# xbpeng/DeepMimic

Measured on NVIDIA H100. Metric: env-steps/sec (30 Hz policy steps; humanoid3d_spinkick, 4096 envs/GPU), higher is better.
Workload: dtype f32

## Files before the change

### deepmimic_b200/csrc/kernels/dm_step.cu

```cuda
#include "dm_model.cuh"
#include <type_traits>

namespace dmk {

namespace {

template <int W>
struct Tl {
    static __device__ __forceinline__ float shfl(float v, int src) { return __shfl_sync(0xffffffffu, v, src, W); }
    static __device__ __forceinline__ int shfli(int v, int src) { return __shfl_sync(0xffffffffu, v, src, W); }
    static __device__ __forceinline__ V3 shfl3(V3 v, int src) { return mk3(shfl(v.x, src), shfl(v.y, src), shfl(v.z, src)); }
    static __device__ __forceinline__ S6 shfl6(S6 v, int src) { return mks(shfl3(v.a, src), shfl3(v.l, src)); }
};
__device__ __forceinline__ void ld12(const float* p, float* o) {
    const float4 a = reinterpret_cast<const float4*>(p)[0], b = reinterpret_cast<const float4*>(p)[1], c_ = reinterpret_cast<const float4*>(p)[2];
    o[0] = a.x; o[1] = a.y; o[2] = a.z; o[3] = a.w; o[4] = b.x; o[5] = b.y; o[6] = b.z; o[7] = b.w; o[8] = c_.x; o[9] = c_.y; o[10] = c_.z; o[11] = c_.w;
}
__device__ __forceinline__ void st12(float* p, const float* o) {
    reinterpret_cast<float4*>(p)[0] = make_float4(o[0], o[1], o[2], o[3]); reinterpret_cast<float4*>(p)[1] = make_float4(o[4], o[5], o[6], o[7]);
    reinterpret_cast<float4*>(p)[2] = make_float4(o[8], o[9], o[10], o[11]);
}
__device__ __forceinline__ float rcp_fast(float x) { float r; asm("rcp.approx.ftz.f32 %0, %1;" : "=f"(r) : "f"(x)); return r; }
__device__ __forceinline__ int wmax(int v) {
#pragma unroll
// ... 31 lines not shown
__device__ __forceinline__ V3 quat_rotvec3(Q4 q) {
    float s = sqrtf(q.x * q.x + q.y * q.y + q.z * q.z);
    if (!(s > 0.000001f)) return mk3(0.f, 0.f, 0.f);
    float th = normalize_angle3(2.0f * atan2f(s, q.w));
    float k = th / s;
    return mk3(q.x * k, q.y * k, q.z * k);
}
__device__ __forceinline__ Q4 quat_integrate3(V3 omega, Q4 quat, bool base_body, float dt) {
    V3 angvel = base_body ? omega : qrot(quat, omega);
    float fAngle = sqrtf(dot(angvel, angvel));
    const float kThr = 0.5f * 1.57079632679489661923f;
    if (fAngle * dt > kThr) fAngle = kThr / dt;
    V3 axis;
    if (fAngle < 0.001f) axis = angvel * __fmaf_rn(-fAngle, (dt * dt * dt) * 0.020833333333f * fAngle, 0.5f * dt);
    else axis = angvel * (__sinf(0.5f * fAngle * dt) / fAngle);
    float cw = __cosf(fAngle * dt * 0.5f);
    Q4 r = base_body ? qmul(quat, mkq(-axis.x, -axis.y, -axis.z, cw)) : qmul(mkq(axis.x, axis.y, axis.z, cw), quat);
    float n = rsqrtf(r.x * r.x + r.y * r.y + r.z * r.z + r.w * r.w);
    return mkq(r.x * n, r.y * n, r.z * n, r.w * n);
}

enum LkSlot { kLC = 0 , kLM = 3,
              kLD = 4 , kLThr = 7,
              kLWd = 8 , kLInt = 14 , kLInt2 = 15 ,
              kLWb = 16 , kLFlg = 22 , kLTree = 23 ,
              kLAx = 24 , kLTl = 27,
              kLZr = 28 ,
              kLHe = 32 , kLKp = 35,
              kLKd = 36, kLLo = 37, kLHi = 38, kLChild = 39 ,
              kLDc = 40 , kLMc = 43 ,
              kLDyn = 44 , kLDChild = 45 ,
              kLkFloats = 48 };
__device__ __forceinline__ float4 ld4(const float* p) { return *reinterpret_cast<const float4*>(p); }
enum HdrSlot { kHLayout = 0, kHLvc = 24, kHGrav = 32 , kHh = 35, kHScale = 36, kHMu = 37, kHFdt = 38, kHDmax = 39 , kHdrFloats = 40 };
__device__ __forceinline__ float* step_smem() { extern __shared__ __align__(16) float dm_step_sm[]; return dm_step_sm; }

}

int dm_step_layout(int nl, int n, int chain_len, int maxrows, int W, StepLayout* L) {
    const int maxpts = maxrows / 3;
    int o = 0;
    L->nl = nl; L->n = n; L->chain_len = chain_len; L->maxrows = maxrows; L->maxpts = maxpts;
    L->oU = o; o += nl * 24;
    L->oR = o; o += nl * 12;
    L->oA = o;
    const int world = nl * 24, tri = maxrows * (maxrows + 1) / 2;
    L->oW = o; L->oV = o + nl * 12;
    L->oPp = o + world; L->oQ = L->oPp + maxpts * 4;
    const int pre = world + maxpts * 4 + 4 * 8;
    o += (pre > tri ? pre : tri);
    o = (o + 3) & ~3;
    const int ys = dm_step_y_stride(W), scr = 28 * (nl - 1);
    L->oY = o; o += (chain_len * ys > scr) ? chain_len * ys : scr;
    L->oLam = o; o += maxrows; o += (o & 1); L->oRhs = o; o += maxrows; L->oInv = o; o += maxrows;
    L->oRl = o; o += maxrows;
    L->oPi = o; o += maxpts; L->oPr = o; o += maxpts;
    L->oG = o; o += 21 + 13 + 2;
    L->oZ = o; o += ((n + 3) / 4) * 4;
    L->env_floats = ((o + 15) / 32) * 32 + 16;
    L->hot_floats = kHdrFloats + ((nl * kLkFloats + (nl * nl + nl * chain_len + 3) / 4 + 3) / 4) * 4;
    return L->hot_floats * 4 + 0;
}
int dm_step_smem_bytes(const StepLayout& L, int tiles) { return (L.hot_floats + L.env_floats * tiles) * static_cast<int>(sizeof(float)); }

constexpr int kSubstepBarriers = 2;
constexpr int kPgsBlock = 2;
enum PgsSection { kSecLimit = 0, kSecNormal = 1, kSecFriction = 2 };
// ... 64 lines not shown
            for (int k = 0; k < B; ++k) ao[s][k] = a_own(s, ik[k], tk[k]);
#pragma unroll
        for (int k = 0; k < B; ++k) {
            float sel = w[0];
#pragma unroll
            for (int s = 1; s < S; ++s) if (ik[k] >= s * W) sel = w[s];
            wk[k] = T::shfl(sel, (S == 1) ? ik[k] : (ik[k] & (W - 1)));
        }
#pragma unroll
        for (int k = 0; k < B; ++k) {
            float c = fmaxf(fmaf(-inv[k], wk[k], rhs[k]), lo[k] - lam[k]);
            if (SEC != kSecNormal) c = fminf(c, hi[k] - lam[k]);
            c = vk[k] ? c : 0.f;
#pragma unroll
            for (int j = k + 1; j < B; ++j) wk[j] = fmaf(ain[j * (j - 1) / 2 + k], c, wk[j]);
            if (vk[k] && writer[k]) sLam[ik[k]] = (SEC == kSecNormal) ? fmaxf(lam[k] + c, 0.f) : fminf(fmaxf(lam[k] + c, lo[k]), hi[k]);
#pragma unroll
            for (int s = 0; s < S; ++s) w[s] = fmaf(ao[s][k], c, w[s]);
        }
        __syncwarp();
    };
#pragma unroll 1
    for (int it = 0; it < 10; ++it) {
#pragma unroll 1
        for (int p0 = 0; p0 < NLmax; p0 += B) block(p0, it, std::integral_constant<int, kSecLimit>{});
#pragma unroll 1
        for (int p0 = 0; p0 < Pmax; p0 += B) block(p0, it, std::integral_constant<int, kSecNormal>{});
#pragma unroll 1
        for (int p0 = 0; p0 < 2 * Pmax; p0 += B) block(p0, it, std::integral_constant<int, kSecFriction>{});
    }
}

template <int W>
__device__ __noinline__ void solve_rows(int NL, int P, float* mani, int alive, unsigned int* prf) {
    using T = Tl<W>;
    float* const sm_ = step_smem();
    const int* LYS = reinterpret_cast<const int*>(sm_ + kHLayout);
    const float* LK = sm_ + kHdrFloats;
    const int lane = threadIdx.x % W;
    const float h = sm_[kHh], mu = sm_[kHMu];
#ifdef DM_PROFILE
    unsigned int pt = static_cast<unsigned int>(clock64());
#define SPROF(sec) do { if ((threadIdx.x & 31) == 0) { unsigned int t_ = static_cast<unsigned int>(clock64()); prf[sec] += t_ - pt; pt = t_; } } while (0)
#else
#define SPROF(sec) do { } while (0)
#endif
    const StepLayout& LY = *reinterpret_cast<const StepLayout*>(LYS);
    const int nl = LY.nl, CL = LY.chain_len, MR = LY.maxrows;
    constexpr int YS = dm_step_y_stride(W);
    float* const E = sm_ + LY.hot_floats + (threadIdx.x / W) * LY.env_floats;
    const unsigned char* CD = reinterpret_cast<const unsigned char*>(LK + nl * kLkFloats);
    const unsigned char* CH = CD + nl * nl;
    float* sU = E + LY.oU; float* sS = E + LY.oR; float* sW = E + LY.oW; float* sV = E + LY.oV; float* sA = E + LY.oA; float* sY = E + LY.oY;
    float* sLam = E + LY.oLam; float2* sRI = reinterpret_cast<float2*>(E + LY.oRhs); int* sRl = reinterpret_cast<int*>(E + LY.oRl);
    float* sPp = E + LY.oPp; float* sPi = E + LY.oPi; int* sPr = reinterpret_cast<int*>(E + LY.oPr);
    float* sQ = E + LY.oQ; float* sG = E + LY.oG; float* sZ = E + LY.oZ;
    auto lk_i = [&](int j) { return reinterpret_cast<const int*>(LK + j * kLkFloats)[kLInt]; };
    auto lk_i2 = [&](int j) { return reinterpret_cast<const int*>(LK + j * kLkFloats)[kLInt2]; };
    auto shift_f = [](S6 f, V3 c) { return mks(f.a + cross(c, f.l), f.l); };
    const int NR = NL + 3 * P;
    const int NRmax = (W == 32) ? NR : wmax(NR);
    const int nslots = (NRmax + W - 1) / W;
    constexpr int kSlots = 2;
#pragma unroll
    for (int s = 0; s < kSlots; ++s) {
        const int rid = lane + s * W;
        if (s < nslots) {
            const bool rv_ = rid < NR;
            int b = 0, kind = 0 , p = 0;
            float lsign = 1.f, lpen = 0.f;
            if (rv_) {
                if (rid < NL) { b = __float_as_int(sQ[rid]); lsign = sQ[8 + rid]; lpen = sQ[16 + rid]; }
                else if (rid < NL + P) { kind = 1; p = rid - NL; b = sPr[p] >> 2; }
                else { const int f = rid - NL - P; p = f >> 1; kind = 2 + (f & 1); b = sPr[p] >> 2; }
                sRl[rid] = b;
            }
            S6 f = mks(mk3(0, 0, 0), mk3(0, 0, 0));
            float rvel = 0.f, pdist = 0.f;
            if (rv_ && kind != 0) {
                const float* w = sW + b * 12;
                pdist = sPp[p * 4 + 3];
                const V3 rel = mk3(sPp[p * 4] - w[9], sPp[p * 4 + 1] - w[10], sPp[p * 4 + 2] - w[11]);
                const V3 fl_ = (kind == 1) ? mk3(0.f, 1.f, 0.f) : ((kind == 2) ? mk3(-1.f, 0.f, 0.f) : mk3(0.f, 0.f, 1.f));
                f = mks(cross(rel, fl_), fl_);
                const float* v = sV + b * 12;
                rvel = dot(fl_, mk3(v[3], v[4], v[5]) + cross(mk3(v[0], v[1], v[2]), rel));
            }
            float acc = 0.f;
            int cur = b;
            bool first = true;
#pragma unroll 1
            while (true) {
                const int info = lk_i(cur);
                const int par = static_cast<int>(static_cast<signed char>(info & 0xff)), nd = (info >> 16) & 0xff, dp0 = (info >> 24) & 0xff;
                const float4* u4 = reinterpret_cast<const float4*>(sU + cur * 24);
                const float4* q4 = reinterpret_cast<const float4*>(sS + cur * 12);
                const float4 ua = u4[0], ub = u4[1], uc = u4[2], ud = u4[3], ue = u4[4], uf = u4[5];
                const float4 qa = q4[0], qb = q4[1], qc = q4[2];
                if (nd == 3) {
// ... 31 lines not shown
            {
                float x[6] = {f.a.x, f.a.y, f.a.z, f.l.x, f.l.y, f.l.z};
                int o = 0;
#pragma unroll
                for (int i = 0; i < 6; ++i) {
#pragma unroll
                    for (int k = 0; k < i; ++k) x[i] -= sG[o++] * x[k];
                    x[i] *= sG[15 + i];
                    if (rv_) sY[i * YS + rid] = x[i];
                    acc += x[i] * x[i];
                }
            }
            if (rv_) {
                const float inv = acc > 1.1920929e-7f ? 1.0f / acc : 0.f;
                float rhs, lam0 = 0.f;
                if (kind == 1) {
                    float perr = 0.f, verr = -rvel;
                    if (pdist > 0.f) verr -= pdist / h; else perr = -pdist * 0.2f / h;
                    rhs = perr * inv + verr * inv;
                    lam0 = sPi[p] * 0.85f;
                } else if (kind != 0) rhs = -rvel * inv;
                else {
                    float perr = 0.f, verr = -rvel;
                    const bool combine = lpen > -0.04f;
                    if (lpen > 0.f) verr = -lpen / h; else perr = -lpen * 0.2f / h;
                    rhs = combine ? (perr * inv + verr * inv) : (verr * inv);
                }
                sRI[rid] = make_float2(rhs, inv); sLam[rid] = lam0;
            }
        }
    }
    __syncwarp();
    SPROF(7);
    const int Pmax = (W == 32) ? P : wmax(P);
    const int NLmax = (W == 32) ? NL : wmax(NL);
    {
        constexpr int kSq2 = (W == 16) ? 22 : 36;
        const int region = max(nl * 24, MR * (MR + 1) / 2);
        const int mode = (nslots == 1) ? 0 : ((NRmax <= kSq2 && kSq2 * kSq2 + W <= region) ? 1 : 2);
        const int st = (mode == 0) ? W : kSq2;
        auto put = [&](int i, int j, float v) {
            if (mode != 2) { sA[i * st + j] = v; sA[j * st + i] = v; }
            else { const int hi_ = max(i, j), lo_ = min(i, j); sA[hi_ * (hi_ + 1) / 2 + lo_] = v; }
        };
#pragma unroll 1
        for (int j = 0; j < NLmax; ++j) {
            const bool jv = j < NL;
            const int bj = jv ? sRl[j] : 0;
#pragma unroll 1
            for (int i0 = 0; i0 < NRmax; i0 += W) {
                const int i = i0 + lane;
                const bool pv = jv && i < NR && i >= j;
                const int cd = pv ? CD[sRl[i] * nl + bj] : 0;
                const float* yi = sY + (pv ? i : 0); const float* yj = sY + (jv ? j : 0);
                float acc = 0.f;
#pragma unroll 1
                for (int k = 0; k < CL; k += 4, yi += 4 * YS, yj += 4 * YS) {
                    const float a0 = yi[0], a1 = yi[YS], a2 = yi[2 * YS], a3 = yi[3 * YS];
                    const float b0 = yj[0], b1 = yj[YS], b2 = yj[2 * YS], b3 = yj[3 * YS];
                    if (k < cd) acc += a0 * b0;
                    if (k + 1 < cd) acc += a1 * b1;
                    if (k + 2 < cd) acc += a2 * b2;
                    if (k + 3 < cd) acc += a3 * b3;
                }
                if (pv) put(i, j, acc);
            }
        }
        const int npp = P * (P + 1) / 2, nppmax = Pmax * (Pmax + 1) / 2;
#pragma unroll 1
        for (int q0 = 0; q0 < nppmax; q0 += W) {
            const int q = q0 + lane;
            const bool pv = q < npp;
            int pp = static_cast<int>((sqrtf(8.0f * static_cast<float>(q) + 1.0f) - 1.0f) * 0.5f);
            if (pp * (pp + 1) / 2 > q) --pp;
            if ((pp + 1) * (pp + 2) / 2 <= q) ++pp;
            const int pr = q - pp * (pp + 1) / 2;
            const int in_p = pv ? NL + pp : 0, it_p = pv ? NL + P + 2 * pp : 0, in_r = pv ? NL + pr : 0, it_r = pv ? NL + P + 2 * pr : 0;
            const int cd = pv ? CD[sRl[in_p] * nl + sRl[in_r]] : 0;
            const float* ypn = sY + in_p; const float* ypt = sY + it_p; const float* yrn = sY + in_r; const float* yrt = sY + it_r;
            float acc[3][3];
#pragma unroll
            for (int x = 0; x < 3; ++x)
#pragma unroll
                for (int y = 0; y < 3; ++y) acc[x][y] = 0.f;
#pragma unroll 1
            for (int k = 0; k < CL; k += 4, ypn += 4 * YS, ypt += 4 * YS, yrn += 4 * YS, yrt += 4 * YS) {
                float av[3][4], bv[3][4];
#pragma unroll
                for (int d = 0; d < 4; ++d) {
                    av[0][d] = ypn[d * YS]; av[1][d] = ypt[d * YS]; av[2][d] = ypt[d * YS + 1];
                    bv[0][d] = yrn[d * YS]; bv[1][d] = yrt[d * YS]; bv[2][d] = yrt[d * YS + 1];
                }
#pragma unroll
                for (int d = 0; d < 4; ++d)
                    if (k + d < cd) {
#pragma unroll
                        for (int x = 0; x < 3; ++x)
#pragma unroll
                            for (int y = 0; y < 3; ++y) acc[x][y] += av[x][d] * bv[y][d];
                    }
            }
            if (pv) {
                if (mode != 2) {
                    float* rp[3] = {sA + in_p * st, sA + it_p * st, sA + it_p * st + st};
                    float* rr[3] = {sA + in_r * st, sA + it_r * st, sA + it_r * st + st};
                    const int cp[3] = {in_p, it_p, it_p + 1}, cr[3] = {in_r, it_r, it_r + 1};
#pragma unroll
                    for (int x = 0; x < 3; ++x)
#pragma unroll
                        for (int y = 0; y < 3; ++y) { rp[x][cr[y]] = acc[x][y]; rr[y][cp[x]] = acc[x][y]; }
                } else {
#pragma unroll
                    for (int x = 0; x < 3; ++x)
#pragma unroll
                        for (int y = 0; y < 3; ++y) put(x == 0 ? in_p : it_p + x - 1, y == 0 ? in_r : it_r + y - 1, acc[x][y]);
                }
            }
        }
        __syncwarp();
        SPROF(8);
        if (mode == 0) pgs_sweeps<W, 1, W, kPgsBlock>(sA, sLam, sRI, lane, NL, P, NLmax, Pmax, mu);
        else if (mode == 1) pgs_sweeps<W, kSlots, kSq2, kPgsBlock>(sA, sLam, sRI, lane, NL, P, NLmax, Pmax, mu);
        else pgs_sweeps<W, kSlots, 0, kPgsBlock>(sA, sLam, sRI, lane, NL, P, NLmax, Pmax, mu);
    }
    SPROF(9);
#pragma unroll 1
    for (int p = lane; p < P; p += W) {
        if (alive) {
            const int ref = sPr[p];
            float* mpt = mani + (ref >> 2) * kManifoldFloats + (ref & 3) * 12;
            mpt[7] = sLam[NL + p]; mpt[8] = sLam[NL + P + 2 * p]; mpt[9] = sLam[NL + P + 2 * p + 1];
        }
    }
    {
        const int info = (lane < nl) ? lk_i(lane) : 0;
        const int nd = (info >> 16) & 0xff, dp0 = (info >> 24) & 0xff;
        const int d0 = (lane < nl) ? (lk_i2(lane) & 0xff) : 0;
        float z0 = 0.f, z1 = 0.f, z2 = 0.f, zb = 0.f;
        const int kb = (lane < 6) ? lane : 0;
        const bool mine = lane < nl && nd > 0;
        const int need = dp0 + nd - 1;
        const unsigned char* cdl = CD + lane;
#pragma unroll 2
        for (int i = 0; i < NRmax; ++i) {
            const int b = sRl[i];
            const float l = (i < NR) ? sLam[i] : 0.f;
            const float yb = sY[kb * YS + i], y0 = sY[dp0 * YS + i], y1 = sY[(dp0 + 1) * YS + i], y2 = sY[(dp0 + 2) * YS + i];
            const bool in = mine && cdl[b * nl] > need;
            zb = fmaf(yb, l, zb);
            if (in) { z0 = fmaf(y0, l, z0); if (nd == 3) { z1 = fmaf(y1, l, z1); z2 = fmaf(y2, l, z2); } }
        }
        if (lane < 6) sZ[lane] = zb;
        if (lane < nl && nd >= 1) sZ[d0] = z0;
        if (lane < nl && nd == 3) { sZ[d0 + 1] = z1; sZ[d0 + 2] = z2; }
    }
    __syncwarp();
}


struct Ctx {
    float* E;
    const int* LYS;
    const float* LK;
    int lane, li;
    int plane, level, ndof, jtype, maxlevel;
    bool act;
};
__device__ __forceinline__ const StepLayout& lay_of(const Ctx& c) { return *reinterpret_cast<const StepLayout*>(c.LYS); }
template <int W>
__device__ __forceinline__ Ctx make_ctx() {
    Ctx c;
    float* sm = step_smem();
    c.LYS = reinterpret_cast<const int*>(sm + kHLayout); c.LK = sm + kHdrFloats;
    const StepLayout& LY = *reinterpret_cast<const StepLayout*>(c.LYS);
    const int tile = threadIdx.x / W;
    c.lane = threadIdx.x % W;
    c.act = c.lane < LY.nl;
    c.li = c.act ? c.lane : LY.nl - 1;
    c.E = sm + LY.hot_floats + tile * LY.env_floats;
    const int* q = reinterpret_cast<const int*>(c.LK + c.li * kLkFloats);
    const int info = q[kLInt], tree = q[kLTree];
    const int par = static_cast<int>(static_cast<signed char>(info & 0xff));
    c.plane = par >= 0 ? par : 0; c.jtype = (info >> 8) & 0xff; c.ndof = c.act ? ((info >> 16) & 0xff) : 0;
    c.level = c.act ? (tree & 0xff) : 1000; c.maxlevel = (tree >> 8) & 0xff;
    return c;
}
__device__ __forceinline__ S6 shift_m(S6 m, V3 c) { return mks(m.a, m.l + cross(m.a, c)); }
__device__ __forceinline__ S6 shift_f(S6 f, V3 c) { return mks(f.a + cross(c, f.l), f.l); }
__device__ __forceinline__ float cl100(float v) { return fminf(fmaxf(v, -100.f), 100.f); }
template <int W>
__device__ __forceinline__ V3 tile_com(const float* w, const float* v, float mass, float inv_total) {
// ... 485 lines not shown
static_assert(dm_step_y_stride(32) / 3 < 32 && dm_step_y_stride(32) < 256, "contact points and solver rows must fit their LoopBits fields");
struct LoopBits {
    unsigned w = 0;
    __device__ __forceinline__ unsigned get(LoopField f) const { return (w >> (f & 31)) & ((1u << (f >> 5)) - 1u); }
    __device__ __forceinline__ void set(LoopField f, unsigned v) { const unsigned m = ((1u << (f >> 5)) - 1u) << (f & 31); w = (w & ~m) | ((v << (f & 31)) & m); }
};
constexpr int kBUpdates = 13;
template <int W>
struct EnvRefs {
    int tid, lane, li, env;
    bool act;
    float* E;
    float* sB;
    const float* LKo;
    float* sim; double* tm; int* fl; float* mani;
    __device__ __forceinline__ EnvRefs(const DevState& st, const StepLayout& LY, int env_id) {
        asm volatile("mov.u32 %0, %%tid.x;" : "=r"(tid));
        env = env_id;
        asm volatile("" : "+r"(env));
        lane = tid % W;
        act = lane < LY.nl;
        li = act ? lane : LY.nl - 1;
        E = step_smem() + LY.hot_floats + (tid / W) * LY.env_floats;
        sB = E + LY.oG + 21;
        LKo = step_smem() + kHdrFloats + li * kLkFloats;
        sim = st.sim + static_cast<size_t>(env) * sim_stride(LY.nl);
        tm = st.time + static_cast<size_t>(env) * kTimeDoubles;
        fl = st.flags + static_cast<size_t>(env) * kFlagInts;
        mani = st.manifold + static_cast<size_t>(env) * LY.nl * kManifoldFloats;
    }
    __device__ __forceinline__ int lk_int(int slot) const { return reinterpret_cast<const int*>(LKo)[slot]; }
};

template <int W, bool TASK>
__global__ void __launch_bounds__(kStepMaxThreads, 1) dm_step_kernel(const DevModel* __restrict__ gm, DevState st, const double* __restrict__ frame_times,
                                                                       const float* __restrict__ frames, double dt, int n_updates, int sim_substeps, StepLayout LY) {
    using T = Tl<W>;
    extern __shared__ __align__(16) float sm[];
    const int tiles = blockDim.x / W;
    const int tile = threadIdx.x / W;
    const int lane = threadIdx.x % W;
    const int slot = blockIdx.x * tiles + tile;
    const int env = (W == 16 && st.order) ? st.order[slot] : slot;
    const DevModel& M = *gm;
    const int nl = LY.nl, CL = LY.chain_len;
    const bool act = lane < nl;
    const int li = act ? lane : nl - 1;

    float* LK = sm + kHdrFloats;
    unsigned char* CD = reinterpret_cast<unsigned char*>(LK + nl * kLkFloats);
    unsigned char* CH = CD + nl * nl;
    int* LYS = reinterpret_cast<int*>(sm + kHLayout);
    for (int j = threadIdx.x; j < nl; j += blockDim.x) {
        const DevLink& K = M.link[j];
        float* q = LK + j * kLkFloats;
        const int p = K.parent;
        for (int k = 0; k < 3; ++k) { q[kLC + k] = K.evec[k] + (p >= 0 ? M.link[p].dvec[k] : 0.f); q[kLD + k] = K.dvec[k]; q[kLAx + k] = K.axis[k]; }
        q[kLM] = K.mass;
        auto lumped = [&](int c_) { const DevLink& C_ = M.link[c_]; return C_.ndof == 0 && C_.nchild == 0 && C_.parent >= 0 && M.link[C_.parent].ndof > 0; };
        const bool isroot = p < 0, self_lumped = lumped(j);
        {
            float cm = 0.f, mdx = 0.f, mdy = 0.f, mdz = 0.f, wD[6] = {0, 0, 0, 0, 0, 0}, wB[6] = {0, 0, 0, 0, 0, 0};
            auto add_part = [&](float m_, V3 r, const float* iD, const float* iB) {
                const float rr = dot(r, r);
                const float sh[6] = {m_ * (rr - r.x * r.x), -m_ * r.x * r.y, -m_ * r.x * r.z, m_ * (rr - r.y * r.y), -m_ * r.y * r.z, m_ * (rr - r.z * r.z)};
                for (int k = 0; k < 6; ++k) { wD[k] += iD[k] + sh[k]; wB[k] += iB[k] + sh[k]; }
// ... 14 lines not shown
                    float rD[6], rB[6];
                    rot_sym(Rc, cD, rD); rot_sym(Rc, cB, rB);
                    add_part(C_.mass, rc, rD, rB);
                }
            }
            for (int k = 0; k < 6; ++k) { q[kLWd + k] = wD[k]; q[kLWb + k] = wB[k]; }
            q[kLMc] = cm;
            const float icm = cm > 0.f ? 1.0f / cm : 0.f;
            q[kLDc] = mdx * icm; q[kLDc + 1] = mdy * icm; q[kLDc + 2] = mdz * icm;
            int dch = 0, dn = 0;
            for (int k = 0; k < K.nchild; ++k) if (!lumped(K.child[k])) { dch |= (K.child[k] & 0xff) << (8 * dn); ++dn; }
            const int dlev = isroot ? -1 : (self_lumped ? 100 : K.level - 1);
            const int dpar = isroot ? 0 : p, byp = (!isroot && p >= 0 && M.link[p].parent < 0) ? p : 0xff;
            reinterpret_cast<int*>(q)[kLDyn] = (dpar & 0xff) | ((dlev & 0xff) << 8) | ((byp & 0xff) << 16) | ((dn & 0xff) << 24);
            reinterpret_cast<int*>(q)[kLDChild] = dch;
        }
        reinterpret_cast<int*>(q)[kLInt] = (K.parent & 0xff) | ((K.jtype & 0xff) << 8) | ((K.ndof & 0xff) << 16) | ((K.depth0 & 0xff) << 24);
        reinterpret_cast<int*>(q)[kLInt2] = (K.dof0 & 0xff) | ((K.last_depth & 0xff) << 8) | ((K.nchild & 0xff) << 16);
        for (int k = 0; k < 4; ++k) q[kLZr + k] = K.zrot[k];
        for (int k = 0; k < 3; ++k) q[kLHe + k] = K.he[k];
        q[kLThr] = K.break_thr; q[kLKp] = K.kp; q[kLKd] = K.kd; q[kLTl] = K.tlim; q[kLLo] = K.lim_lo; q[kLHi] = K.lim_hi;
        reinterpret_cast<int*>(q)[kLFlg] = (K.shape & 0xff) | ((K.fall_contact & 0xff) << 8) | ((K.has_limit & 0xff) << 16);
        reinterpret_cast<int*>(q)[kLTree] = (K.level & 0xff) | ((M.maxlevel & 0xff) << 8) | ((K.nchild & 0xff) << 16);
        reinterpret_cast<int*>(q)[kLChild] = (K.child[0] & 0xff) | ((K.child[1] & 0xff) << 8) | ((K.child[2] & 0xff) << 16) | ((K.child[3] & 0xff) << 24);
        for (int d = 0; d < CL; ++d) CH[j * CL + d] = M.chain_dof[j][d];
        for (int b = 0; b < nl; ++b) {
            int cnt = 0;
            const int lim = min(K.last_depth, M.link[b].last_depth);
            while (cnt <= lim && M.chain_dof[j][cnt] == M.chain_dof[b][cnt]) ++cnt;
            CD[j * nl + b] = static_cast<unsigned char>(cnt);
        }
    }
    if (threadIdx.x == blockDim.x - 1) {
        static_assert(sizeof(StepLayout) / sizeof(int) <= kHLvc, "StepLayout must fit the header slot");
        const int* src = reinterpret_cast<const int*>(&LY);
        for (int k = 0; k < static_cast<int>(sizeof(StepLayout) / sizeof(int)); ++k) LYS[k] = src[k];
        sm[kHGrav] = M.gravity[0]; sm[kHGrav + 1] = M.gravity[1]; sm[kHGrav + 2] = M.gravity[2];
        sm[kHh] = static_cast<float>(dt) / static_cast<float>(sim_substeps); sm[kHScale] = M.scale; sm[kHMu] = M.friction; sm[kHFdt] = static_cast<float>(dt);
    }
    if (threadIdx.x == 8) {
        int mx = 0;
        for (int j = 0; j < nl; ++j) { const DevLink& K = M.link[j]; if (K.parent >= 0 && !(K.ndof == 0 && K.nchild == 0 && M.link[K.parent].ndof > 0)) mx = max(mx, K.level - 1); }
        reinterpret_cast<int*>(sm)[kHDmax] = mx;
    }
    __syncthreads();

    float4 jp, jv;
    LoopBits ls;
    {
        const EnvRefs<W> r(st, LY, env);
        for (int k = lane * 4; k < LY.env_floats; k += W * 4) *reinterpret_cast<float4*>(r.E + k) = make_float4(0.f, 0.f, 0.f, 0.f);
        __syncwarp();
        float* sB = r.sB;
        const float* sim = r.sim;
        if (lane == 0) {
            float4 b0 = reinterpret_cast<const float4*>(sim)[0], b1 = reinterpret_cast<const float4*>(sim)[1], b2 = reinterpret_cast<const float4*>(sim)[2],
                   b3 = reinterpret_cast<const float4*>(sim)[3];
            sB[0] = b0.x; sB[1] = b0.y; sB[2] = b0.z; sB[3] = b1.x; sB[4] = b1.y; sB[5] = b1.z; sB[6] = b1.w;
            sB[7] = b2.x; sB[8] = b2.y; sB[9] = b2.z; sB[10] = b3.x; sB[11] = b3.y; sB[12] = b3.z;
            reinterpret_cast<int*>(sB)[kBUpdates] = r.fl[kFUpdates];
        }
        jp = reinterpret_cast<const float4*>(sim + 16)[li];
        jv = reinterpret_cast<const float4*>(sim + 16 + 4 * nl)[li];
        ls.set(kLsNeedAction, r.fl[kFNeedAction] != 0);
        ls.set(kLsAlive, r.fl[kFDone] == 0);
        ls.set(kLsOver, r.fl[kFRowOverflow] != 0);
        ls.set(kLsNeedKin, 1);
// ... 91 lines not shown
                task_fail = T::shfli(tf, 0);
                fallen_eff = T::shfli(fe, 0);
            }
            if (ls.get(kLsAlive)) {
                int term = (M.enable_fall_end && fallen_eff) ? 1 : 0;
                if (!term && (ls.get(kLsClock) & 4)) term = 1;
                if (TASK && !term && task_fail) term = task_fail;
                if (lane == 0) ++reinterpret_cast<int*>(sB)[kBUpdates];
                const bool end = (ls.get(kLsClock) & 2) || term;
                if (end || stage == total_stages) {
                    float* sim = r.sim; int* fl = r.fl;
                    if (lane == 0) {
                        reinterpret_cast<float4*>(sim)[0] = make_float4(sB[0], sB[1], sB[2], 0.f);
                        reinterpret_cast<float4*>(sim)[1] = make_float4(sB[3], sB[4], sB[5], sB[6]);
                        reinterpret_cast<float4*>(sim)[2] = make_float4(sB[7], sB[8], sB[9], 0.f);
                        reinterpret_cast<float4*>(sim)[3] = make_float4(sB[10], sB[11], sB[12], 0.f);
                        fl[kFNeedAction] = ls.get(kLsNeedAction); fl[kFDone] = end ? 1 : 0; fl[kFTerminate] = term; fl[kFValid] = (eseg == 0) ? 1 : 0; fl[kFFallen] = fallen_eff;
                        fl[kFRowOverflow] = ls.get(kLsOver); fl[kFUpdates] = reinterpret_cast<const int*>(sB)[kBUpdates];
                        if (W == 16) st.load[r.env] = ls.get(kLsRows);
                    }
                    if (act) {
                        reinterpret_cast<float4*>(sim + 16)[lane] = jp;
                        reinterpret_cast<float4*>(sim + 16 + 4 * nl)[lane] = jv;
                    }
                }
                if (end) ls.set(kLsAlive, 0);
            }
        }
        PROF(1);
        if (stage == total_stages) break;
        if (__syncthreads_and(!ls.get(kLsAlive))) break;
        PROF(2);
        if (__ballot_sync(0xffffffffu, ls.get(kLsAlive)) == 0u) {
            if ((stage % stages_per_upd) != 0)
                for (int k = 0; k < kSubstepBarriers; ++k) __syncthreads();
            continue;
        }
        const int ph = stage % stages_per_upd;
        if (ph == 0) {
            const EnvRefs<W> r(st, LY, env);
            const int lane = r.lane, li = r.li;
            float* sB = r.sB;
            int cb = 0;
            if constexpr (TASK) {
                if (__ballot_sync(0xffffffffu, ls.get(kLsAlive) && ls.get(kLsNeedAction)) != 0u) {
                    const float scale = step_smem()[kHScale];
                    const V3 com = tile_com<W>(r.E + LY.oW + li * 12, r.E + LY.oV + li * 12, r.act ? r.LKo[kLM] : 0.f, 1.0f / (M.total_mass * scale));
                    double* tk = st.task + static_cast<size_t>(r.env) * kTaskDoubles;
                    if (lane == 0 && ls.get(kLsAlive) && ls.get(kLsNeedAction)) { tk[kKPrevCom] = com.x; tk[kKPrevCom + 1] = com.y; tk[kKPrevCom + 2] = com.z; }
                }
            }
            if (lane == 0 && ls.get(kLsAlive)) {
                double* tm = r.tm;
                const double timer = tm[kTTimer] + dt;
                double kin_time = tm[kTKin];
                double dur_ = M.motion_dur;
                if constexpr (TASK) dur_ = st.ctab->info[st.clip[r.env]].dur;
                const double dur = dur_;
                double p0 = kin_time / dur; p0 -= floor(p0);
                kin_time += dt;
                double p1 = kin_time / dur; p1 -= floor(p1);
                if constexpr (TASK) {
                    const ClipInfo& ci = st.ctab->info[st.clip[r.env]];
                    if (ci.loop && p1 < p0 && M.sync_root_pos) {
                        const double simq[4] = {static_cast<double>(sB[3]), static_cast<double>(sB[4]), static_cast<double>(sB[5]), static_cast<double>(sB[6])};
                        kin_wrap_sync(frame_times + ci.frame_off, frames + static_cast<size_t>(ci.frame_off) * M.pose_dim, M.pose_dim, ci.num_frames, ci.cycle_delta, dur, kin_time,
                                      tm + kTOrigin, tm + kTOriginRot, static_cast<double>(sB[0]) / M.scale, static_cast<double>(sB[2]) / M.scale, simq, true, false);
                    }
// ... 40 lines not shown
            const float fdt = step_smem()[kHFdt], kd = r2.LKo[kLKd];
            const int ndof = r2.act ? ((r2.lk_int(kLInt) >> 16) & 0xff) : 0;
            float t0 = 0, t1 = 0, t2 = 0;
            if (ndof >= 1) t0 = pe0 + kd * (-jv.x - fdt * qdd.x);
            if (ndof == 3) { t1 = pe1 + kd * (-jv.y - fdt * qdd.y); t2 = pe2 + kd * (-jv.z - fdt * qdd.z); }
            const float mag = sqrtf(t0 * t0 + t1 * t1 + t2 * t2), tlim = r2.LKo[kLTl];
            if (mag > tlim) { float s = tlim / mag; t0 *= s; t1 *= s; t2 *= s; }
            tau0 = t0; tau1 = t1; tau2 = t2;
            PROF(4);
            continue;
        }
        if (ph == sim_substeps) ls.set(kLsPendingFlags, 1);
        {
            const int r = collide<W>(EnvRefs<W>(st, LY, env).mani, ls.get(kLsAlive) ? 1 : 0, ls.get(kLsMcnt));
            ls.set(kLsNpts, r & 0xff); ls.set(kLsContactTol, (r >> 8) & 1); if ((r >> 9) & 1) ls.set(kLsOver, 1); ls.set(kLsMcnt, (r >> 10) & 7);
        }
        PROF(3);
        {
            const float3 qdd = aba_solve<W>(tau0, tau1, tau2, 0.f, 1, jv.x, jv.y, jv.z);
            const EnvRefs<W> r(st, LY, env);
            const float h = step_smem()[kHh];
            const int ndof = r.act ? ((r.lk_int(kLInt) >> 16) & 0xff) : 0;
            bool hit = false;
            if (ndof >= 1) { const float v = jv.x + h * qdd.x; jv.x = cl100(v); hit |= fabsf(v) > 100.f; }
            if (ndof == 3) { const float v1 = jv.y + h * qdd.y, v2 = jv.z + h * qdd.z; jv.y = cl100(v1); jv.z = cl100(v2); hit |= fabsf(v1) > 100.f || fabsf(v2) > 100.f; }
            if (r.lane == 0) for (int k = 0; k < 6; ++k) hit |= fabsf(r.sB[7 + k]) >= 100.f;
            const unsigned hb = __ballot_sync(0xffffffffu, hit);
            if (hb != 0u) {
                const unsigned hseg = (W == 32) ? hb : ((hb >> (r.tid & 16)) & 0xffffu);
                vel_pass<W>(jv.x, jv.y, jv.z, hseg != 0u);
            }
        }
        PROF(ph == 1 ? 16 : 17);
        __syncthreads();
        PROF(2);
        int lim_dir = 0; float lim_pen = 0.f;
        const EnvRefs<W> r(st, LY, env);
        const bool has_limit = ((r.lk_int(kLFlg) >> 16) & 0xff) != 0;
        if (r.act && has_limit && ls.get(kLsAlive)) {
            float p0 = jp.x - r.LKo[kLLo], p1 = r.LKo[kLHi] - jp.x;
            if (!(p0 > 0.f)) { lim_dir = 1; lim_pen = p0; }
            else if (!(p1 > 0.f)) { lim_dir = -1; lim_pen = p1; }
        }
        const unsigned lbal = __ballot_sync(0xffffffffu, lim_dir != 0);
        const unsigned lseg = (W == 32) ? lbal : ((lbal >> (r.tid & 16)) & 0xffffu);
        int NL = __popc(lseg);
        int P = ls.get(kLsNpts);
        const unsigned anyrow = __ballot_sync(0xffffffffu, NL + P > 0);
        ls.set(kLsRows, 0);
        if (anyrow != 0) {
            {
                const int lidx = __popc(lseg & ((1u << r.lane) - 1u));
                if (NL > 8) { NL = 8; ls.set(kLsOver, 1); }
                float* sQ = r.E + LY.oQ;
                if (lim_dir != 0 && lidx < 8) { sQ[lidx] = __int_as_float(r.lane); sQ[8 + lidx] = (lim_dir == -1) ? -1.f : 1.f; sQ[16 + lidx] = lim_pen; sQ[24 + lidx] = jv.x; }
            }
            if (NL + 3 * P > LY.maxrows) { P = (LY.maxrows - NL) / 3; ls.set(kLsOver, 1); }
            const int NR = NL + 3 * P;
            ls.set(kLsRows, NR);
            __syncwarp();
            PROF(5);
#ifdef DM_PROFILE
            { const int nrm = wmax(NR); if ((threadIdx.x & 31) == 0) { PRF[13] += nrm; PRF[14] += 1; if (nrm > W) PRF[15] += 1; } }
#endif
            solve_rows<W>(NL, P, r.mani, ls.get(kLsAlive) ? 1 : 0, PRFP);
            PROF(10);
            const float3 dq = dv_pass<W>();
            if (ls.get(kLsRows) > 0) {
                const EnvRefs<W> r2(st, LY, env);
                const int ndof = r2.act ? ((r2.lk_int(kLInt) >> 16) & 0xff) : 0;
                if (ndof >= 1) jv.x = cl100(jv.x + dq.x);
                if (ndof == 3) { jv.y = cl100(jv.y + dq.y); jv.z = cl100(jv.z + dq.z); }
            }
            PROF(11);
        }
        __syncthreads();
        PROF(2);
        const EnvRefs<W> r3(st, LY, env);
        const float h = step_smem()[kHh];
        const int jtype = (r3.lk_int(kLInt) >> 8) & 0xff;
        if (r3.lane == 0) {
            float* sB = r3.sB;
            sB[0] += h * sB[10]; sB[1] += h * sB[11]; sB[2] += h * sB[12];
            const Q4 q = quat_integrate3(mk3(sB[7], sB[8], sB[9]), mkq(sB[3], sB[4], sB[5], sB[6]), true, h);
            sB[3] = q.x; sB[4] = q.y; sB[5] = q.z; sB[6] = q.w;
        }
        if (jtype == kJRevolute) jp.x += h * jv.x;
        else if (jtype == kJSpherical) { Q4 q = quat_integrate3(mk3(jv.x, jv.y, jv.z), mkq(jp.x, jp.y, jp.z, jp.w), false, h); jp = make_float4(q.x, q.y, q.z, q.w); }
        __syncwarp();
        ls.set(kLsNeedKin, 1);
        PROF(12);
    }
#ifdef DM_PROFILE
    __syncwarp();
    if ((threadIdx.x & 31) == 0 && st.prof) { unsigned int* o = st.prof + (blockIdx.x * (blockDim.x / 32) + threadIdx.x / 32) * kProfCounters; for (int k = 0; k < kProfCounters; ++k) o[k] = PRF[k]; }
#endif
}

const StepKernel kStepKernels[2][2] = {{dm_step_kernel<16, false>, dm_step_kernel<16, true>}, {dm_step_kernel<32, false>, dm_step_kernel<32, true>}};
// ... 70 lines not shown
```

Before: 2.772 million.

## Pair heavy-contact warps with idle warps for wide 32-lane row solves

In the half-warp (W=16) mode, each warp publishes its row counts to a shared header table. A matching step then pairs warps whose envs have more rows than fit in 16 lanes with warps that have no rows. Each such pair solves the constraint rows with full 32-lane tiles, synchronised by named barriers, and the owning warp alone then accumulates the z vector. The goal is to cut the serialized two-slot PGS work for heavy-contact envs, at the cost of an extra block barrier, a header re-layout and more complex control flow.

```diff
diff --git a/deepmimic_b200/csrc/kernels/dm_step.cu b/deepmimic_b200/csrc/kernels/dm_step.cu
--- a/deepmimic_b200/csrc/kernels/dm_step.cu
+++ b/deepmimic_b200/csrc/kernels/dm_step.cu
@@ -87,7 +87,10 @@
               kLDyn = 44 , kLDChild = 45 ,
               kLkFloats = 48 };
 __device__ __forceinline__ float4 ld4(const float* p) { return *reinterpret_cast<const float4*>(p); }
-enum HdrSlot { kHLayout = 0, kHLvc = 24, kHGrav = 32 , kHh = 35, kHScale = 36, kHMu = 37, kHFdt = 38, kHDmax = 39 , kHdrFloats = 40 };
+enum HdrSlot { kHLayout = 0, kHGrav = 24 , kHh = 27, kHScale = 28, kHMu = 29, kHFdt = 30, kHDmax = 31 ,
+               kHRows = 32 , kHdrFloats = 48 };
+constexpr int kRowAlive = 64, kHelperOf = 16;
+static_assert(kHRows + kStepMaxThreads / 32 <= kHdrFloats && kHdrFloats % 4 == 0, "the row table must fit the header, which keeps the link table 16-byte aligned");
 __device__ __forceinline__ float* step_smem() { extern __shared__ __align__(16) float dm_step_sm[]; return dm_step_sm; }
 
 }
@@ -218,12 +221,15 @@
 }
 
 template <int W>
-__device__ __noinline__ void solve_rows(int NL, int P, float* mani, int alive, unsigned int* prf) {
-    using T = Tl<W>;
+__device__ __forceinline__ void rows_to_z(const float* E, int lane, int NR, int NRmax);
+template <int W, bool WIDE>
+__device__ __forceinline__ void solve_rows_body(int NL, int P, float* mani, int alive, unsigned int* prf, int tile) {
+    constexpr int LW = WIDE ? 32 : W;
+    using T = Tl<LW>;
     float* const sm_ = step_smem();
     const int* LYS = reinterpret_cast<const int*>(sm_ + kHLayout);
     const float* LK = sm_ + kHdrFloats;
-    const int lane = threadIdx.x % W;
+    const int lane = threadIdx.x % LW;
     const float h = sm_[kHh], mu = sm_[kHMu];
 #ifdef DM_PROFILE
     unsigned int pt = static_cast<unsigned int>(clock64());
@@ -234,7 +240,7 @@
     const StepLayout& LY = *reinterpret_cast<const StepLayout*>(LYS);
     const int nl = LY.nl, CL = LY.chain_len, MR = LY.maxrows;
     constexpr int YS = dm_step_y_stride(W);
-    float* const E = sm_ + LY.hot_floats + (threadIdx.x / W) * LY.env_floats;
+    float* const E = WIDE ? sm_ + LY.hot_floats + tile * LY.env_floats : sm_ + LY.hot_floats + (threadIdx.x / W) * LY.env_floats;
     const unsigned char* CD = reinterpret_cast<const unsigned char*>(LK + nl * kLkFloats);
     const unsigned char* CH = CD + nl * nl;
     float* sU = E + LY.oU; float* sS = E + LY.oR; float* sW = E + LY.oW; float* sV = E + LY.oV; float* sA = E + LY.oA; float* sY = E + LY.oY;
@@ -245,12 +251,13 @@
     auto lk_i2 = [&](int j) { return reinterpret_cast<const int*>(LK + j * kLkFloats)[kLInt2]; };
     auto shift_f = [](S6 f, V3 c) { return mks(f.a + cross(c, f.l), f.l); };
     const int NR = NL + 3 * P;
-    const int NRmax = (W == 32) ? NR : wmax(NR);
-    const int nslots = (NRmax + W - 1) / W;
-    constexpr int kSlots = 2;
+    const int NRmax = (LW == 32) ? NR : wmax(NR);
+    const int nslots = (NRmax + LW - 1) / LW;
+    constexpr int kSlots = WIDE ? 1 : 2;
+    constexpr int kSq2 = (W == 16) ? 22 : 36;
 #pragma unroll
     for (int s = 0; s < kSlots; ++s) {
-        const int rid = lane + s * W;
+        const int rid = lane + s * LW;
         if (s < nslots) {
             const bool rv_ = rid < NR;
             int b = 0, kind = 0 , p = 0;
@@ -348,12 +355,11 @@
     }
     __syncwarp();
     SPROF(7);
-    const int Pmax = (W == 32) ? P : wmax(P);
-    const int NLmax = (W == 32) ? NL : wmax(NL);
+    const int Pmax = (LW == 32) ? P : wmax(P);
+    const int NLmax = (LW == 32) ? NL : wmax(NL);
     {
-        constexpr int kSq2 = (W == 16) ? 22 : 36;
         const int region = max(nl * 24, MR * (MR + 1) / 2);
-        const int mode = (nslots == 1) ? 0 : ((NRmax <= kSq2 && kSq2 * kSq2 + W <= region) ? 1 : 2);
+        const int mode = (nslots == 1 && !WIDE) ? 0 : ((NRmax <= kSq2 && kSq2 * kSq2 + LW <= region) ? 1 : 2);
         const int st = (mode == 0) ? W : kSq2;
         auto put = [&](int i, int j, float v) {
             if (mode != 2) { sA[i * st + j] = v; sA[j * st + i] = v; }
@@ -364,7 +370,7 @@
             const bool jv = j < NL;
             const int bj = jv ? sRl[j] : 0;
 #pragma unroll 1
-            for (int i0 = 0; i0 < NRmax; i0 += W) {
+            for (int i0 = 0; i0 < NRmax; i0 += LW) {
                 const int i = i0 + lane;
                 const bool pv = jv && i < NR && i >= j;
                 const int cd = pv ? CD[sRl[i] * nl + bj] : 0;
@@ -384,7 +390,7 @@
         }
         const int npp = P * (P + 1) / 2, nppmax = Pmax * (Pmax + 1) / 2;
 #pragma unroll 1
-        for (int q0 = 0; q0 < nppmax; q0 += W) {
+        for (int q0 = 0; q0 < nppmax; q0 += LW) {
             const int q = q0 + lane;
             const bool pv = q < npp;
             int pp = static_cast<int>((sqrtf(8.0f * static_cast<float>(q) + 1.0f) - 1.0f) * 0.5f);
@@ -435,44 +441,96 @@
         }
         __syncwarp();
         SPROF(8);
-        if (mode == 0) pgs_sweeps<W, 1, W, kPgsBlock>(sA, sLam, sRI, lane, NL, P, NLmax, Pmax, mu);
-        else if (mode == 1) pgs_sweeps<W, kSlots, kSq2, kPgsBlock>(sA, sLam, sRI, lane, NL, P, NLmax, Pmax, mu);
-        else pgs_sweeps<W, kSlots, 0, kPgsBlock>(sA, sLam, sRI, lane, NL, P, NLmax, Pmax, mu);
+        if (mode == 0 && !WIDE) pgs_sweeps<W, 1, W, kPgsBlock>(sA, sLam, sRI, lane, NL, P, NLmax, Pmax, mu);
+        else if (mode == 1) pgs_sweeps<LW, kSlots, kSq2, kPgsBlock>(sA, sLam, sRI, lane, NL, P, NLmax, Pmax, mu);
+        else pgs_sweeps<LW, kSlots, 0, kPgsBlock>(sA, sLam, sRI, lane, NL, P, NLmax, Pmax, mu);
     }
     SPROF(9);
 #pragma unroll 1
-    for (int p = lane; p < P; p += W) {
+    for (int p = lane; p < P; p += LW) {
         if (alive) {
             const int ref = sPr[p];
             float* mpt = mani + (ref >> 2) * kManifoldFloats + (ref & 3) * 12;
             mpt[7] = sLam[NL + p]; mpt[8] = sLam[NL + P + 2 * p]; mpt[9] = sLam[NL + P + 2 * p + 1];
         }
     }
-    {
-        const int info = (lane < nl) ? lk_i(lane) : 0;
-        const int nd = (info >> 16) & 0xff, dp0 = (info >> 24) & 0xff;
-        const int d0 = (lane < nl) ? (lk_i2(lane) & 0xff) : 0;
-        float z0 = 0.f, z1 = 0.f, z2 = 0.f, zb = 0.f;
-        const int kb = (lane < 6) ? lane : 0;
-        const bool mine = lane < nl && nd > 0;
-        const int need = dp0 + nd - 1;
-        const unsigned char* cdl = CD + lane;
+    if (WIDE) {
+        asm volatile("bar.sync %0, 64;" ::"r"(tile / 2 + 1) : "memory");
+        if (tile & 1) return;
+        const int e = reinterpret_cast<const int*>(sm_)[kHRows + tile / 2], sh = (threadIdx.x & 16) ? 16 : 8;
+        rows_to_z<W>(sm_ + LY.hot_floats + static_cast<int>(threadIdx.x / W) * LY.env_floats, threadIdx.x % W, ((e >> sh) & 15) + 3 * ((e >> (sh + 4)) & 15), e & 63);
+        return;
+    }
+    const int info = (lane < nl) ? lk_i(lane) : 0;
+    const int nd = (info >> 16) & 0xff, dp0 = (info >> 24) & 0xff;
+    const int d0 = (lane < nl) ? (lk_i2(lane) & 0xff) : 0;
+    float z0 = 0.f, z1 = 0.f, z2 = 0.f, zb = 0.f;
+    const int kb = (lane < 6) ? lane : 0;
+    const bool mine = lane < nl && nd > 0;
+    const int need = dp0 + nd - 1;
+    const unsigned char* cdl = CD + lane;
 #pragma unroll 2
-        for (int i = 0; i < NRmax; ++i) {
-            const int b = sRl[i];
-            const float l = (i < NR) ? sLam[i] : 0.f;
-            const float yb = sY[kb * YS + i], y0 = sY[dp0 * YS + i], y1 = sY[(dp0 + 1) * YS + i], y2 = sY[(dp0 + 2) * YS + i];
-            const bool in = mine && cdl[b * nl] > need;
-            zb = fmaf(yb, l, zb);
-            if (in) { z0 = fmaf(y0, l, z0); if (nd == 3) { z1 = fmaf(y1, l, z1); z2 = fmaf(y2, l, z2); } }
-        }
-        if (lane < 6) sZ[lane] = zb;
-        if (lane < nl && nd >= 1) sZ[d0] = z0;
-        if (lane < nl && nd == 3) { sZ[d0 + 1] = z1; sZ[d0 + 2] = z2; }
-    }
+    for (int i = 0; i < NRmax; ++i) {
+        const int b = sRl[i];
+        const float l = (i < NR) ? sLam[i] : 0.f;
+        const float yb = sY[kb * YS + i], y0 = sY[dp0 * YS + i], y1 = sY[(dp0 + 1) * YS + i], y2 = sY[(dp0 + 2) * YS + i];
+        const bool in = mine && cdl[b * nl] > need;
+        zb = fmaf(yb, l, zb);
+        if (in) { z0 = fmaf(y0, l, z0); if (nd == 3) { z1 = fmaf(y1, l, z1); z2 = fmaf(y2, l, z2); } }
+    }
+    if (lane < 6) sZ[lane] = zb;
+    if (lane < nl && nd >= 1) sZ[d0] = z0;
+    if (lane < nl && nd == 3) { sZ[d0 + 1] = z1; sZ[d0 + 2] = z2; }
     __syncwarp();
 }
-
+template <int W>
+__device__ __noinline__ void solve_rows(int NL, int P, float* mani, int alive, unsigned int* prf) { solve_rows_body<W, false>(NL, P, mani, alive, prf, 0); }
+template <int W>
+__device__ __noinline__ void solve_rows_wide(int pm, float* manifold, const int* order, unsigned int* prf) {
+    const float* sm_ = step_smem();
+    const StepLayout& LY = *reinterpret_cast<const StepLayout*>(sm_ + kHLayout);
+    const bool helper = pm >= kHelperOf;
+    const int tile = helper ? 2 * (pm - kHelperOf) + 1 : static_cast<int>(threadIdx.x / 32) * 2;
+    const int e = reinterpret_cast<const int*>(sm_)[kHRows + tile / 2], sh = helper ? 16 : 8;
+    const int slot = blockIdx.x * (blockDim.x / W) + tile;
+    float* const mani = manifold + static_cast<size_t>(order ? order[slot] : slot) * LY.nl * kManifoldFloats;
+    solve_rows_body<W, true>((e >> sh) & 15, (e >> (sh + 4)) & 15, mani, 1, prf, tile);
+}
+
+template <int W>
+__device__ __forceinline__ void rows_to_z(const float* E, int lane, int NR, int NRmax) {
+    const float* sm_ = step_smem();
+    const StepLayout& LY = *reinterpret_cast<const StepLayout*>(sm_ + kHLayout);
+    const float* LK = sm_ + kHdrFloats;
+    const int nl = LY.nl;
+    constexpr int YS = dm_step_y_stride(W);
+    const unsigned char* CD = reinterpret_cast<const unsigned char*>(LK + nl * kLkFloats);
+    const float* sY = E + LY.oY; const float* sLam = E + LY.oLam; const int* sRl = reinterpret_cast<const int*>(E + LY.oRl);
+    float* sZ = const_cast<float*>(E) + LY.oZ;
+    auto lk_i = [&](int j) { return reinterpret_cast<const int*>(LK + j * kLkFloats)[kLInt]; };
+    auto lk_i2 = [&](int j) { return reinterpret_cast<const int*>(LK + j * kLkFloats)[kLInt2]; };
+    const int info = (lane < nl) ? lk_i(lane) : 0;
+    const int nd = (info >> 16) & 0xff, dp0 = (info >> 24) & 0xff;
+    const int d0 = (lane < nl) ? (lk_i2(lane) & 0xff) : 0;
+    float z0 = 0.f, z1 = 0.f, z2 = 0.f, zb = 0.f;
+    const int kb = (lane < 6) ? lane : 0;
+    const bool mine = lane < nl && nd > 0;
+    const int need = dp0 + nd - 1;
+    const unsigned char* cdl = CD + lane;
+#pragma unroll 2
+    for (int i = 0; i < NRmax; ++i) {
+        const int b = sRl[i];
+        const float l = (i < NR) ? sLam[i] : 0.f;
+        const float yb = sY[kb * YS + i], y0 = sY[dp0 * YS + i], y1 = sY[(dp0 + 1) * YS + i], y2 = sY[(dp0 + 2) * YS + i];
+        const bool in = mine && cdl[b * nl] > need;
+        zb = fmaf(yb, l, zb);
+        if (in) { z0 = fmaf(y0, l, z0); if (nd == 3) { z1 = fmaf(y1, l, z1); z2 = fmaf(y2, l, z2); } }
+    }
+    if (lane < 6) sZ[lane] = zb;
+    if (lane < nl && nd >= 1) sZ[d0] = z0;
+    if (lane < nl && nd == 3) { sZ[d0 + 1] = z1; sZ[d0 + 2] = z2; }
+    __syncwarp();
+}
 
 struct Ctx {
     float* E;
@@ -1024,6 +1082,37 @@
     __device__ __forceinline__ int lk_int(int slot) const { return reinterpret_cast<const int*>(LKo)[slot]; }
 };
 
+__device__ __forceinline__ int pair_match(const int* tab, int nw, int w, int W) {
+    unsigned heavy = 0u, idle = 0u;
+#pragma unroll 1
+    for (int k = 0; k < nw; ++k) {
+        const int e = tab[k];
+        if (e & kRowAlive) { if ((e & 63) > W) heavy |= 1u << k; else if ((e & 63) == 0) idle |= 1u << k; }
+    }
+    if ((heavy >> w) & 1u) {
+        int rank = __popc(heavy & ((1u << w) - 1u));
+        if (rank >= __popc(idle)) return -1;
+        for (; rank > 0; --rank) idle &= ~(0x80000000u >> __clz(idle));
+        return 31 - __clz(idle);
+    }
+    if ((idle >> w) & 1u) {
+        int rank = __popc(idle >> (w + 1));
+        if (rank >= __popc(heavy)) return -1;
+        for (; rank > 0; --rank) heavy &= heavy - 1u;
+        return kHelperOf + __ffs(heavy) - 1;
+    }
+    return -1;
+}
+__device__ __forceinline__ int opaque_tid() { int v; asm volatile("mov.u32 %0, %%tid.x;" : "=r"(v)); return v; }
+__device__ __forceinline__ int opaque_ntid() { int v; asm volatile("mov.u32 %0, %%ntid.x;" : "=r"(v)); return v; }
+template <int W>
+__device__ __forceinline__ float* tile_manifold(const DevState& st, const StepLayout& LY, int tile) {
+    int cta; asm volatile("mov.u32 %0, %%ctaid.x;" : "=r"(cta));
+    const int slot = cta * (opaque_ntid() / W) + tile;
+    const int env = (W == 16 && st.order) ? st.order[slot] : slot;
+    return st.manifold + static_cast<size_t>(env) * LY.nl * kManifoldFloats;
+}
+
 template <int W, bool TASK>
 __global__ void __launch_bounds__(kStepMaxThreads, 1) dm_step_kernel(const DevModel* __restrict__ gm, DevState st, const double* __restrict__ frame_times,
                                                                        const float* __restrict__ frames, double dt, int n_updates, int sim_substeps, StepLayout LY) {
@@ -1104,7 +1193,7 @@
         }
     }
     if (threadIdx.x == blockDim.x - 1) {
-        static_assert(sizeof(StepLayout) / sizeof(int) <= kHLvc, "StepLayout must fit the header slot");
+        static_assert(sizeof(StepLayout) / sizeof(int) <= kHGrav, "StepLayout must fit the header slot");
         const int* src = reinterpret_cast<const int*>(&LY);
         for (int k = 0; k < static_cast<int>(sizeof(StepLayout) / sizeof(int)); ++k) LYS[k] = src[k];
         sm[kHGrav] = M.gravity[0]; sm[kHGrav + 1] = M.gravity[1]; sm[kHGrav + 2] = M.gravity[2];
@@ -1262,8 +1351,10 @@
         if (__syncthreads_and(!ls.get(kLsAlive))) break;
         PROF(2);
         if (__ballot_sync(0xffffffffu, ls.get(kLsAlive)) == 0u) {
-            if ((stage % stages_per_upd) != 0)
+            if ((stage % stages_per_upd) != 0) {
+                if (W == 16 && (threadIdx.x & 31) == 0) reinterpret_cast<int*>(sm)[kHRows + threadIdx.x / 32] = 0;
                 for (int k = 0; k < kSubstepBarriers; ++k) __syncthreads();
+            }
             continue;
         }
         const int ph = stage % stages_per_upd;
@@ -1370,8 +1461,6 @@
             }
         }
         PROF(ph == 1 ? 16 : 17);
-        __syncthreads();
-        PROF(2);
         int lim_dir = 0; float lim_pen = 0.f;
         const EnvRefs<W> r(st, LY, env);
         const bool has_limit = ((r.lk_int(kLFlg) >> 16) & 0xff) != 0;
@@ -1394,15 +1483,24 @@
                 if (lim_dir != 0 && lidx < 8) { sQ[lidx] = __int_as_float(r.lane); sQ[8 + lidx] = (lim_dir == -1) ? -1.f : 1.f; sQ[16 + lidx] = lim_pen; sQ[24 + lidx] = jv.x; }
             }
             if (NL + 3 * P > LY.maxrows) { P = (LY.maxrows - NL) / 3; ls.set(kLsOver, 1); }
-            const int NR = NL + 3 * P;
-            ls.set(kLsRows, NR);
-            __syncwarp();
-            PROF(5);
+            ls.set(kLsRows, NL + 3 * P);
+        }
+        if constexpr (W == 16) {
+            const int nrm = wmax(NL + 3 * P), nl1 = __shfl_sync(0xffffffffu, NL, 16), p1 = __shfl_sync(0xffffffffu, P, 16);
+            if ((r.tid & 31) == 0) reinterpret_cast<int*>(sm)[kHRows + r.tid / 32] = nrm | kRowAlive | (NL << 8) | (P << 12) | (nl1 << 16) | (p1 << 20);
+        }
+        __syncwarp();
+        PROF(5);
+        __syncthreads();
+        PROF(2);
+        const int pm = (W == 16) ? pair_match(reinterpret_cast<const int*>(sm) + kHRows, opaque_ntid() / 32, opaque_tid() / 32, W) : -1;
 #ifdef DM_PROFILE
-            { const int nrm = wmax(NR); if ((threadIdx.x & 31) == 0) { PRF[13] += nrm; PRF[14] += 1; if (nrm > W) PRF[15] += 1; } }
+        if (anyrow != 0) { const int nrm = wmax(NL + 3 * P); if ((threadIdx.x & 31) == 0) { PRF[13] += nrm; PRF[14] += 1; if (nrm > W) PRF[15] += 1; if (pm >= 0) PRF[6] += 1; } }
 #endif
-            solve_rows<W>(NL, P, r.mani, ls.get(kLsAlive) ? 1 : 0, PRFP);
-            PROF(10);
+        if (__ballot_sync(0xffffffffu, pm >= 0) != 0u) solve_rows_wide<W>(pm, st.manifold, st.order, PRFP);
+        else if (anyrow != 0) solve_rows<W>(NL, P, r.mani, ls.get(kLsAlive) ? 1 : 0, PRFP);
+        PROF(10);
+        if (__ballot_sync(0xffffffffu, ls.get(kLsRows) > 0) != 0u) {
             const float3 dq = dv_pass<W>();
             if (ls.get(kLsRows) > 0) {
                 const EnvRefs<W> r2(st, LY, env);
```

After: 2.845 million, median of 6. 2.6% higher.
